# fab-jul/imgcomp-cvpr

Measured on AMD Instinct MI355X. Metric: Megapixels/s encode+pc-logits (and decode) per node, higher is better.
Workload: dtype f32

## Files before the change

### imgcomp_cvpr_amd/_lib.py

```python
import ctypes
import os
from ctypes import c_char_p, c_float, c_int, c_int64, c_longlong, c_size_t, c_uint32, c_void_p, POINTER

_HERE = os.path.dirname(os.path.abspath(__file__))
LIB_PATH = os.environ.get('IMGCOMP_HIP_LIB') or os.path.join(_HERE, 'libimgcomp_hip.so')


class HipLibraryError(RuntimeError):
    pass


CONV3_FORM_MASK = 0x0f
CONV3_AUTO, CONV3_DIRECT, CONV3_WINO, CONV3_WINO_WHOLEK, CONV3_WINO_WHOLEK_PW = 0, 1, 2, 3, 4
CONV3_WINO_KSPLIT, CONV3_WINO_T16, CONV3_WINO_SEG1, CONV3_WINO_SEG2, CONV3_WINO_SEG3 = 5, 6, 7, 8, 9
CONV3_WINO_PAIR = 10
CONV3_WINO4 = 11
CONV3_NO_WINO4 = 0x800000
CONV3_WINO4_WG8 = 0x8000000
CONV3_WINO4_WG4 = 0x10000000
CONV5_BOTH_PACKED = 0x1000000
CONV5_WINO4 = 0x2000000
CONV5_NO_WINO4 = 0x4000000
CONV3_LEAVE_IDLE_CUS = 0x10
CONV3_NO_XCD_RUNS = 0x20
CONV3_PACKED_TRANSFORM = 0x40
CONV3_STACK_KERNEL = 0x80


def CONV3_IN_FLIGHT(n):
    return (min(int(n), 15) & 0xf) << 19
PC_DECODE_PER_LAYER = 0x01
PC_DECODE_RECOMPUTE = 0x02
PC_DECODE_WAVEFRONT = 0x04


def conv3_leave_idle_layers(n):
    return (n & 0x7f) << 12


def conv3_direct_variant(v):
    return ((v + 1) & 0xf) << 8


def edge_tiles_per_wg(n):
    return n & 0xff


class PcTile(ctypes.Structure):
    _fields_ = [('y0', c_int), ('x0', c_int), ('th', c_int), ('tw', c_int), ('stream_off', c_longlong), ('stream_bytes', c_longlong),
                ('first_sym', c_int), ('volume', c_int)]


class PcVolume(ctypes.Structure):
    _fields_ = [('h', c_int), ('w', c_int), ('symbols_off', c_longlong), ('q_off', c_longlong)]


class PcSeg(ctypes.Structure):
    _fields_ = [('off', c_longlong), ('nbytes', c_longlong)]


def seg_table(segs):
    arr = (PcSeg * max(len(segs), 1))()
    for i, (off, n) in enumerate(segs):
        arr[i] = PcSeg(int(off), int(n))
    return arr


def tile_table(tiles):
    arr = (PcTile * len(tiles))()
    for i, t in enumerate(tiles):
        t = [int(v) for v in t]
        arr[i] = PcTile(*(t if len(t) == 8 else t + [0]))
    return arr


def volume_table(volumes):
    arr = (PcVolume * len(volumes))()
    for i, v in enumerate(volumes):
        arr[i] = PcVolume(*[int(x) for x in v])
    return arr


def packed_volume_table(shapes):
    offs, total = [], 0
    for C, h, w in shapes:
        offs.append(total)
        total += int(C) * int(h) * int(w)
    return volume_table([(h, w, o, o) for (C, h, w), o in zip(shapes, offs)]), offs, total


PROTOTYPES = {
    'ic_abi_version': (c_int, []),
    'ic_strerror': (c_char_p, [c_int]),
    'ic_crc32c': (c_uint32, [c_void_p, c_size_t, c_uint32]),
    'ic_conv2d_bn_act_f32': (c_int, [c_void_p] * 7 + [c_int] * 9 + [c_void_p, c_void_p, c_void_p]),
    'ic_deconv2d_bn_act_f32': (c_int, [c_void_p] * 5 + [c_int] * 8 + [c_void_p, c_void_p, c_int, c_void_p]),
    'ic_conv3x3_c128_packed_floats': (c_size_t, []),
    'ic_pack_conv3x3_c128_f32': (c_int, [c_void_p, c_void_p, c_void_p]),
    'ic_conv3x3_c128_bn_act_f32': (c_int, [c_void_p] * 7 + [c_int] * 5 + [c_void_p]),
    'ic_wino3x3_c128_packed_floats': (c_size_t, []),
    'ic_pack_wino3x3_c128_f32': (c_int, [c_void_p, c_void_p, c_int, c_void_p]),
    'ic_pack_wino3x3_c128_batch_f32': (c_int, [c_void_p, c_void_p, c_int, c_int, c_void_p]),
    'ic_wino3x3_c128_bn_act_f32': (c_int, [c_void_p] * 7 + [c_int] * 5 + [c_void_p]),
    'ic_wino3x3_c128_workgroups': (c_longlong, [c_int, c_int, c_int, c_int]),
    'ic_wino3x3_c128_plan': (c_int, [c_int, c_int, c_int, c_int, POINTER(c_longlong)]),
    'ic_conv3x3_c128_both_packed_floats': (c_size_t, []),
    'ic_pack_conv3x3_c128_both_f32': (c_int, [c_void_p, c_void_p, c_int, c_void_p]),
    'ic_conv3x3_c128_pick_algo': (c_int, [c_int, c_int, c_int, c_int]),
    'ic_conv3x3_c128_auto_f32': (c_int, [c_void_p] * 7 + [c_int] * 5 + [c_void_p]),
    'ic_conv2d_mfma_packed_floats': (c_size_t, [c_int] * 6),
    'ic_pack_conv2d_mfma_f32': (c_int, [c_void_p, c_void_p] + [c_int] * 6 + [c_void_p]),
    'ic_conv2d_mfma_bn_act_f32': (c_int, [c_void_p] * 5 + [c_int] * 10 + [c_void_p]),
    'ic_quantize_f32': (c_int, [c_void_p, c_void_p, c_int, c_float, c_void_p, c_void_p, c_void_p,
                                c_longlong, c_void_p]),
    'ic_heatmap_quantize_f32': (c_int, [c_void_p, c_void_p, c_int, c_float] + [c_void_p] * 6 +
                                [c_int] * 4 + [c_void_p]),
    'ic_pc_workspace_bytes': (c_size_t, [c_int] * 5),
    'ic_pc_packed_floats': (c_size_t, [c_int, c_int]),
    'ic_pc_mid_tile': (c_int, [c_int, c_int, c_int]),
    'ic_pc_pack_filters_f32': (c_int, [POINTER(c_void_p), c_int, c_int, c_void_p, c_void_p]),
    'ic_pc_logits_f32': (c_int, [c_void_p, POINTER(c_void_p), c_int, c_int, c_float, c_void_p] +
                         [c_int] * 4 + [c_void_p, c_size_t, c_void_p]),
    'ic_pc_logits_padded_f32': (c_int, [c_void_p, POINTER(c_void_p), c_int, c_int, c_void_p] +
                                [c_int] * 4 + [c_void_p, c_size_t, c_void_p]),
    'ic_pc_bitcost_f32': (c_int, [c_void_p, c_void_p, POINTER(c_void_p), c_int, c_int, c_float,
                                  c_void_p, c_void_p] + [c_int] * 4 + [c_void_p, c_size_t, c_void_p]),
    'ic_pc_logits_to_freqs_f32': (c_int, [c_void_p, c_longlong, c_int, c_float, c_void_p, c_void_p, c_void_p]),
    'ic_pc_encode_capacity_bytes': (c_size_t, [c_longlong]),
    'ic_pc_encode_f32': (c_int, [c_void_p, c_void_p, c_int, c_longlong, c_int, c_float, c_void_p, c_longlong, c_void_p, c_void_p,
                                 c_void_p]),
    'ic_pc_decode_workspace_bytes': (c_size_t, [c_int] * 4),
    'ic_pc_decode_f32': (c_int, [c_void_p, c_longlong, c_int, POINTER(c_void_p), c_void_p, c_int, c_int, c_float,
                                 c_void_p, c_void_p, c_int, c_int, c_int, c_void_p, c_size_t, c_int, c_void_p]),
    'ic_pc_decode_tiles_workspace_bytes': (c_size_t, [c_int] * 5),
    'ic_pc_decode_tiles_f32': (c_int, [c_void_p, c_longlong, c_void_p, c_int, POINTER(c_void_p), c_void_p, c_int, c_int, c_float,
                                       c_void_p, c_void_p, c_int, c_int, c_int, c_void_p, c_size_t, c_int, c_void_p]),
    'ic_pc_decode_tiles_batch_workspace_bytes': (c_size_t, [c_int] * 6),
    'ic_pc_decode_tiles_batch_f32': (c_int, [c_void_p, c_longlong, c_void_p, c_int, c_void_p, c_int, POINTER(c_void_p), c_void_p, c_int,
                                             c_int, c_float, c_void_p, c_void_p, c_void_p, c_int, c_void_p, c_size_t, c_int, c_void_p]),
    'ic_pc_decode_channels_f32': (c_int, [c_void_p, c_longlong, c_int, POINTER(c_void_p), c_void_p, c_int, c_int, c_float,
                                          c_void_p, c_void_p, c_int, c_int, c_int, c_void_p, c_size_t, c_int, c_void_p, c_int, c_int]),
    'ic_pc_decode_tiles_batch_channels_f32': (c_int, [c_void_p, c_longlong, c_void_p, c_int, c_void_p, c_int, POINTER(c_void_p), c_void_p,
                                                      c_int, c_int, c_float, c_void_p, c_void_p, c_void_p, c_int, c_void_p, c_size_t,
                                                      c_int, c_void_p, c_int, c_int]),
    'ic_pc_decode_tiles_batch_layers_workspace_bytes': (c_size_t, [c_int] * 7),
    'ic_pc_decode_tiles_batch_layers_f32': (c_int, [c_void_p, c_longlong, c_void_p, c_int, c_void_p, c_int, POINTER(c_void_p), c_void_p,
                                                    c_int, c_int, c_float, c_void_p, c_void_p, c_void_p, c_int, c_void_p, c_size_t,
                                                    c_int, c_void_p, c_int, c_int, c_void_p, c_int, c_void_p]),
    'ic_pc_encode_segments_f32': (c_int, [c_void_p, c_void_p, c_int, c_longlong, c_int, c_float, c_void_p, c_int, c_void_p, c_longlong,
                                          c_void_p, c_void_p, c_void_p]),
    'ic_pc_conceal_tiles_workspace_bytes': (c_size_t, [c_int, c_int, c_longlong]),
    'ic_pc_conceal_tiles': (c_int, [c_void_p, c_void_p, c_void_p, c_int, c_void_p, c_int, c_void_p, c_void_p] + [c_int] * 5 +
                            [c_void_p, c_size_t, c_void_p]),
    'ic_sum_f32': (c_int, [c_void_p, c_longlong, c_void_p, c_void_p, c_void_p]),
    'ic_mean_f32': (c_int, [c_void_p, c_longlong, c_float, c_void_p, c_void_p, c_void_p]),
    'ic_mean_rows_f32': (c_int, [c_void_p, c_int, c_longlong, c_float, c_void_p, c_void_p, c_void_p]),
    'ic_ae_workspace_bytes': (c_size_t, [c_int] * 4),
    'ic_ae_sync_pos_bytes': (c_size_t, [c_int] * 4),
    'ic_ae_res_stack_sync_pos_bytes': (c_size_t, [c_int] * 3),
    'ic_ae_encode_f32': (c_int, [c_void_p, POINTER(c_void_p)] + [c_int] * 5 + [c_void_p] * 6 +
                         [c_int] * 3 + [c_void_p, c_size_t, c_int, c_void_p]),
    'ic_ae_decode_f32': (c_int, [c_void_p, POINTER(c_void_p)] + [c_int] * 3 + [c_void_p] +
                         [c_int] * 3 + [c_void_p, c_size_t, c_int, c_void_p]),
    'ic_ae_res_stack_workspace_bytes': (c_size_t, [c_int] * 3),
    'ic_ae_res_stack_f32': (c_int, [c_void_p, POINTER(c_void_p), c_int, c_void_p] + [c_int] * 3 + [c_void_p, c_size_t, c_int, c_void_p]),
    'ic_peer_region_bytes': (c_size_t, []),
    'ic_peer_max_values': (c_int, []),
    'ic_peer_max_world': (c_int, []),
    'ic_peer_region_create': (c_int, [c_void_p, c_void_p]),
    'ic_peer_region_open': (c_int, [c_void_p, c_void_p]),
    'ic_peer_region_close': (c_int, [c_void_p]),
    'ic_peer_region_destroy': (c_int, [c_void_p]),
    'ic_peer_allreduce_f64': (c_int, [c_void_p, c_int, c_void_p, c_int, c_int, c_uint32, c_void_p, c_void_p]),
    'ic_build_has_tuning_forms': (c_int, []),
    'ic_conv3x3_c128_pick_form': (c_int, [c_int, c_int, c_int, c_int]),
    'ic_wino4_3x3_c128_packed_floats': (c_size_t, []),
    'ic_pack_wino4_3x3_c128_f32': (c_int, [c_void_p, c_void_p, c_int, c_void_p]),
    'ic_pack_wino4_3x3_c128_batch_f32': (c_int, [c_void_p, c_void_p, c_int, c_int, c_void_p]),
    'ic_wino4_3x3_c128_supported': (c_int, [c_int, c_int, c_int]),
# ... 116 lines not shown
```

### imgcomp_cvpr_amd/csrc/conv_edge.hip

```cpp
#include "internal.h"
#include <algorithm>

#define DE_TX 32
#define DE_TY 8

template <int CO>
__global__ __launch_bounds__(256) void deconv5_small_cout_kernel(const ConvArgs a) {
    extern __shared__ __attribute__((aligned(16))) float wl[];
    const int tid = threadIdx.x;
    const int n = blockIdx.z;
    for (int e = tid; e < a.Cin * 25 * 4; e += 256) {
        const int co = e & 3, tap = (e >> 2) % 25, ci = e / 100;
        wl[e] = co < a.Cout ? a.w[((size_t)tap * a.Cout + co) * a.Cin + ci] : 0.f;
    }
    __syncthreads();
    const int qx = blockIdx.x * DE_TX + (tid & (DE_TX - 1));
    const int qy = blockIdx.y * DE_TY + tid / DE_TX;
    const bool live = qx < a.W && qy < a.H;
    const int cx = min(qx, a.W - 1), cy = min(qy, a.H - 1);
    const int HW = a.H * a.W;
    const float* __restrict__ xin = a.x + (size_t)n * a.Cin * HW;
    int noff[9];
    bool nok[9];
#pragma unroll
// ... 112 lines not shown

#pragma unroll
    for (int c = 0; c < NCH; ++c) {
        e_f32x4 A[9][4];
#pragma unroll
        for (int t = 0; t < 9; ++t)
#pragma unroll
            for (int q = 0; q < 4; ++q)
                A[t][q] = *reinterpret_cast<const e_f32x4*>(wl + (size_t)t * 128 * CIN + 32 * c + 4 * q);
        if (c == 0) __syncthreads();
        float bv[2][4];
        auto views = [&](int s, int buf) __attribute__((always_inline)) {
            const float* Ls = L + (32 * c + s) * D3_CS;
            bv[buf][0] = Ls[0]; bv[buf][1] = Ls[-1]; bv[buf][2] = Ls[-D3_S]; bv[buf][3] = Ls[-D3_S - 1];
        };
        views(0, 0);
#pragma unroll
        for (int s = 0; s < 16; ++s) {
            if (s + 1 < 16) views(s + 1, (s + 1) & 1);
            const float b00 = bv[s & 1][0], b0m = bv[s & 1][1], bm0 = bv[s & 1][2], bmm = bv[s & 1][3];
#define D3_A(t) A[t][s >> 2][s & 3]
            p00a = __builtin_amdgcn_mfma_f32_32x32x2f32(D3_A(0), b00, p00a, 0, 0, 0);
            p01 = __builtin_amdgcn_mfma_f32_32x32x2f32(D3_A(1), b00, p01, 0, 0, 0);
            p10 = __builtin_amdgcn_mfma_f32_32x32x2f32(D3_A(3), b00, p10, 0, 0, 0);
            p11 = __builtin_amdgcn_mfma_f32_32x32x2f32(D3_A(4), b00, p11, 0, 0, 0);
            p00b = __builtin_amdgcn_mfma_f32_32x32x2f32(D3_A(2), b0m, p00b, 0, 0, 0);
            p10 = __builtin_amdgcn_mfma_f32_32x32x2f32(D3_A(5), b0m, p10, 0, 0, 0);
            p00a = __builtin_amdgcn_mfma_f32_32x32x2f32(D3_A(6), bm0, p00a, 0, 0, 0);
            p01 = __builtin_amdgcn_mfma_f32_32x32x2f32(D3_A(7), bm0, p01, 0, 0, 0);
            p00b = __builtin_amdgcn_mfma_f32_32x32x2f32(D3_A(8), bmm, p00b, 0, 0, 0);
#undef D3_A
#pragma unroll
            for (int i = 0; i < 9; ++i) {
                __builtin_amdgcn_sched_group_barrier(0x008, 1, 0);
                if (i < 4 && s + 1 < 16) __builtin_amdgcn_sched_group_barrier(0x100, 1, 0);
            }
        }
        __builtin_amdgcn_sched_barrier(0);
    }

    const int gy = gy0 + j / D3_TC, gx = gx0 + j % D3_TC;
    if (gy >= a.H || gx >= a.W) return;
    const size_t ohw = (size_t)a.OH * a.OW;
    float* __restrict__ yb = a.y + ((size_t)n * a.Cout + 32 * wave + 4 * kh) * ohw + (size_t)(2 * gy) * a.OW + 2 * gx;
    const float* __restrict__ scp = a.scale + 32 * wave + 4 * kh;
    const float* __restrict__ shp = a.shift + 32 * wave + 4 * kh;
#pragma unroll
    for (int r = 0; r < 16; ++r) {
        const int crow = (r & 3) + 8 * (r >> 2);
        const float sc = scp[crow], sh = shp[crow];
        float2 o0, o1;
        o0.x = fmaf(p00a[r] + p00b[r], sc, sh); o0.y = fmaf(p01[r], sc, sh);
        o1.x = fmaf(p10[r], sc, sh); o1.y = fmaf(p11[r], sc, sh);
        if (a.relu) {
            o0.x = fmaxf(o0.x, 0.f); o0.y = fmaxf(o0.y, 0.f); o1.x = fmaxf(o1.x, 0.f); o1.y = fmaxf(o1.y, 0.f);
        }
        float* dst = yb + (size_t)crow * ohw;
        *reinterpret_cast<float2*>(dst) = o0;
        *reinterpret_cast<float2*>(dst + a.OW) = o1;
    }
}

int icx_deconv3_mfma(const ConvArgs& a, hipStream_t st) {
    if (a.KH != 3 || a.KW != 3 || a.Cout != 128 || a.pt != 0 || a.pl != 0 || a.res1 || a.res2 || a.in_mean ||
        a.out_mean || a.builtin_norm || a.w_sci != 1 || a.w_sco != a.Cin)
        return IC_ERR_UNSUPPORTED;
    if ((long long)a.Cin * a.H * a.W >= (1ll << 31)) return IC_ERR_UNSUPPORTED;
    const int tiles_x = ic_cdiv(a.W, D3_TC), tiles_y = ic_cdiv(a.H, D3_TR);
    const dim3 g((unsigned)(tiles_x * tiles_y * a.N));
    if (a.Cin == 32) hipLaunchKernelGGL((deconv3_mfma_kernel<32>), g, dim3(256), 0, st, a, tiles_x, tiles_y);
    else if (a.Cin == 64) hipLaunchKernelGGL((deconv3_mfma_kernel<64>), g, dim3(256), 0, st, a, tiles_x, tiles_y);
    else return IC_ERR_UNSUPPORTED;
    IC_LAUNCH_CHECK();
    return IC_OK;
}

#define H1_TR 4
#define H1_TC 32
#define H1_ROWS ((H1_TR - 1) * 2 + 6)
#define H1_COLS ((H1_TC - 1) * 2 + 5)
#define H1_HALF ((H1_COLS + 1) / 2)
#define H1_S (2 * H1_HALF)
#define H1_CS (H1_ROWS * H1_S)

__global__ __launch_bounds__(256) void conv5s2_cin3_mfma_kernel(const ConvArgs a, int tiles_x, int tiles_y) {
    constexpr int NE = 3 * H1_ROWS * H1_COLS, NST = (NE + 255) / 256;
    __shared__ float lds[3 * H1_CS];
    __shared__ __attribute__((aligned(16))) float wl[25 * 3 * 64];
    const int tid = threadIdx.x, lane = tid & 63, wave = tid >> 6;
    int b = ic_xcd_run(blockIdx.x, gridDim.x);
    const int tx = b % tiles_x; b /= tiles_x;
    const int ty = b % tiles_y; const int n = b / tiles_y;
    const int ox0 = tx * H1_TC, oy0 = ty * H1_TR;
    const int HW = a.H * a.W;
    const float* __restrict__ xin = a.x + (size_t)n * 3 * HW;
    const int iy0 = 2 * oy0 - a.pt, ix0 = 2 * ox0 - a.pl;
    const bool norm_in = a.in_mean != nullptr || (a.builtin_norm & 1);

#pragma unroll
    for (int i = 0; i < NST; ++i) {
        const int e = tid + 256 * i;
        const int ci = e / (H1_ROWS * H1_COLS), rem = e - ci * (H1_ROWS * H1_COLS);
        const int rr = rem / H1_COLS, cc = rem - rr * H1_COLS;
        const int iy = iy0 + rr, ix = ix0 + cc;
        const bool live = e < NE;
        const bool ok = live && iy >= 0 && iy < a.H && ix >= 0 && ix < a.W;
        float v = xin[ok ? ci * HW + iy * a.W + ix : 0];
        if (norm_in) {
            const int cm = live ? ci : 0;
            const float m = a.in_mean ? a.in_mean[cm] : IC_IMG_MEAN[cm];
            const float s = a.in_mean ? a.in_std[cm] : IC_IMG_STD[cm];
            v = (v - m) / s;
        }
        if (live) lds[ci * H1_CS + rr * H1_S + (cc & 1) * H1_HALF + (cc >> 1)] = ok ? v : 0.f;
    }

    for (int e = tid; e < 25 * 3 * 64 / 4; e += 256)
        reinterpret_cast<float4*>(wl)[e] = reinterpret_cast<const float4*>(a.w)[e];
    __syncthreads();

    const int j = lane & 31, kh = lane >> 5;
    const float* __restrict__ L = lds + (2 * wave + kh) * H1_S + j;
    e_f32x16 acc0, acc1;
#pragma unroll
    for (int r = 0; r < 16; ++r) { acc0[r] = 0.f; acc1[r] = 0.f; }
    float fa[2][2], fb[2];
    auto operands = [&](int s, int buf) __attribute__((always_inline)) {
        const int ci = s / 15, p = (s / 5) % 3, kx = s % 5;
        const int ky = 2 * p + kh;
        const float* wp = wl + (((p < 2 ? ky : 4) * 5 + kx) * 3 + ci) * 64 + j;
        const float w0 = wp[0], w1 = wp[32];
        fa[buf][0] = (p < 2 || kh == 0) ? w0 : 0.f;
        fa[buf][1] = (p < 2 || kh == 0) ? w1 : 0.f;
        fb[buf] = L[ci * H1_CS + 2 * p * H1_S + (kx & 1) * H1_HALF + (kx >> 1)];
    };
    operands(0, 0);
#pragma unroll
    for (int s = 0; s < 45; ++s) {
        if (s + 1 < 45) operands(s + 1, (s + 1) & 1);
        acc0 = __builtin_amdgcn_mfma_f32_32x32x2f32(fa[s & 1][0], fb[s & 1], acc0, 0, 0, 0);
        acc1 = __builtin_amdgcn_mfma_f32_32x32x2f32(fa[s & 1][1], fb[s & 1], acc1, 0, 0, 0);
        __builtin_amdgcn_sched_group_barrier(0x008, 1, 0);
        __builtin_amdgcn_sched_group_barrier(0x100, 2, 0);
        __builtin_amdgcn_sched_group_barrier(0x008, 1, 0);
        __builtin_amdgcn_sched_group_barrier(0x100, 1, 0);
        __builtin_amdgcn_sched_group_barrier(0x002, 2, 0);
    }
    __builtin_amdgcn_sched_barrier(0);

    const int gy = oy0 + wave, gx = ox0 + j;
    if (gy >= a.OH || gx >= a.OW) return;
    const size_t ohw = (size_t)a.OH * a.OW;
    const size_t cs = a.out_phases ? ohw / 4 : ohw;
    const size_t o0 = a.out_phases ? (((size_t)n * 4 + 2 * (gy & 1) + (gx & 1)) * 64 + 4 * kh) * cs + (size_t)(gy >> 1) * (a.OW >> 1) + (gx >> 1)
                                   : ((size_t)n * 64 + 4 * kh) * ohw + (size_t)gy * a.OW + gx;
#pragma unroll
    for (int t = 0; t < 2; ++t)
#pragma unroll
        for (int r = 0; r < 16; ++r) {
            const int co = 32 * t + (r & 3) + 8 * (r >> 2);
            float v = fmaf(t ? acc1[r] : acc0[r], a.scale[co + 4 * kh], a.shift[co + 4 * kh]);
            if (a.relu) v = fmaxf(v, 0.f);
            const size_t o = o0 + (size_t)co * cs;
            if (a.res1) v += a.res1[o];
            if (a.res2) v += a.res2[o];
            a.y[o] = v;
        }
}

int icx_conv5s2_cin3_mfma(const ConvArgs& a, hipStream_t st) {
    if (a.KH != 5 || a.KW != 5 || a.stride != 2 || a.Cin != 3 || a.Cout != 64 || a.w_sco != 1 || a.w_sci != 64 ||
        a.out_mean || (a.builtin_norm & ~1))
        return IC_ERR_UNSUPPORTED;
    if ((long long)a.H * a.W * 3 >= (1ll << 31)) return IC_ERR_UNSUPPORTED;
    if (a.out_phases && ((a.OH | a.OW) & 1 || a.res1 || a.res2)) return IC_ERR_UNSUPPORTED;
    const int tiles_x = ic_cdiv(a.OW, H1_TC), tiles_y = ic_cdiv(a.OH, H1_TR);
    hipLaunchKernelGGL(conv5s2_cin3_mfma_kernel, dim3((unsigned)(tiles_x * tiles_y * a.N)), dim3(256), 0, st, a, tiles_x,
                       tiles_y);
    IC_LAUNCH_CHECK();
    return IC_OK;
}

typedef float e_f32x4v __attribute__((ext_vector_type(4)));
#define H13_TR 8
#define H13_TC 16
#define H13_S (H13_TC + 8)
#define H13_CS ((H13_TR + 2) * H13_S)
#define H13_KC 16
#define H13_UNITS (H13_KC * (H13_TR + 2) * (H13_S / 4))

__global__ __launch_bounds__(256) void deconv5_cout3_mfma_kernel(const ConvArgs a, int tiles_x, int tiles_y, int tpw,
                                                                 unsigned long long* prof) {
#ifdef H13_PROF
    unsigned long long tq[8], tp[4];
    tq[0] = __builtin_amdgcn_s_memtime();
#endif
    constexpr int NCH = 64 / H13_KC;
    constexpr unsigned OOB = 0x80000000u;
    __shared__ float af[16 * 9 * 64];
    __shared__ __attribute__((aligned(16))) float tl[2][H13_KC * H13_CS];
    const int tid = threadIdx.x, lane = tid & 63;
    const int wave = __builtin_amdgcn_readfirstlane(tid >> 6);
    const int strips = (tiles_x + tpw - 1) / tpw;
    int b = ic_xcd_run(blockIdx.x, gridDim.x);
    const int sx = b % strips; b /= strips;
    const int ty = b % tiles_y; const int n = b / tiles_y;
    const int tx0 = sx * tpw, nt = min(tpw, tiles_x - tx0);
    const int gy0 = ty * H13_TR;
    const int HW = a.H * a.W;
    const int j = lane & 15, kg = lane >> 4;
#ifdef H13_PROF
    __builtin_amdgcn_sched_barrier(0);
    tp[3] = __builtin_amdgcn_s_memtime() + (unsigned long long)(nt + HW == -12345);
    __builtin_amdgcn_sched_barrier(0);
#endif
    const __amdgpu_buffer_rsrc_t xr =
        __builtin_amdgcn_make_buffer_rsrc((void*)(a.x + (size_t)n * 64 * HW), 0, 64 * HW * 4, 0x00020000);
    const __amdgpu_buffer_rsrc_t wr = __builtin_amdgcn_make_buffer_rsrc((void*)a.w, 0, 25 * a.Cout * 64 * 4, 0x00020000);

    constexpr int NU = (H13_UNITS + 255) / 256;
    int ubase[NU], ulds[NU], ucol[NU];
#pragma unroll
    for (int i = 0; i < NU; ++i) {
        const int u = tid + 256 * i;
        const int sl = u / 60, rem = u - sl * 60;
        const int row = rem / 6, q = rem - row * 6;
        const int iy = gy0 - 1 + row;
        const bool ok = u < H13_UNITS && iy >= 0 && iy < a.H;
        ubase[i] = ok ? (16 * (sl & 3) + (sl >> 2)) * HW + iy * a.W : -1;
        ucol[i] = 4 * q - 4;
        ulds[i] = u < H13_UNITS ? sl * H13_CS + row * H13_S + 4 * q : -1;
    }
    unsigned voff[NU], vmask = 0;
    auto tile_off = [&](int gx0) {
        vmask = 0;
#pragma unroll
        for (int i = 0; i < NU; ++i) {
            const int ix = gx0 + ucol[i];
            voff[i] = ubase[i] >= 0 && ix >= 0 && ix < a.W ? (unsigned)(ubase[i] + ix) * 4u : OOB;
            const int left = a.W - ix;
            vmask |= (left >= 4 ? 15u : (1u << max(left, 0)) - 1u) << (4 * i);
        }
    };
    auto request = [&](e_f32x4* dst, int chunk) {
        const int cb = chunk * 4 * HW * 4;
#pragma unroll
        for (int i = 0; i < NU; ++i) dst[i] = __builtin_bit_cast(e_f32x4, __builtin_amdgcn_raw_buffer_load_b128(xr, voff[i], cb, 0));
    };
    auto deposit = [&](float* dstl, const e_f32x4* src, unsigned m) {
#pragma unroll
        for (int i = 0; i < NU; ++i) {
            e_f32x4 v = src[i];
#pragma unroll
            for (int e = 0; e < 4; ++e) v[e] = (m >> (4 * i + e)) & 1 ? v[e] : 0.f;
            if (i + 1 < NU || ulds[i] >= 0) *reinterpret_cast<e_f32x4*>(dstl + ulds[i]) = v;
        }
    };

    e_f32x4 fv[9];
    {
        const int i = lane & 15, co = i >> 2, py = (i >> 1) & 1, px = i & 1;
        const int tapf = a.Cout * 64;
        const unsigned lbase = co < a.Cout ? (unsigned)((((py + 1) * 5 + px + 1) * a.Cout + co) * 64 + 16 * kg + 4 * wave) * 4u : OOB;
// ... 158 lines not shown
```

### include/imgcomp_hip.h

```cpp
#ifndef IMGCOMP_HIP_H
#define IMGCOMP_HIP_H

#include <stddef.h>
#include <stdint.h>

#ifdef __cplusplus
extern "C" {
#endif

#define IC_ABI_VERSION 2

#define IC_OK 0
#define IC_ERR_ARG (-1)
#define IC_ERR_UNSUPPORTED (-2)
#define IC_ERR_WORKSPACE (-3)

typedef void* ic_stream_t;

#define IC_CONV3_FORM_MASK        0x0f
#define IC_CONV3_AUTO             0x00
#define IC_CONV3_DIRECT           0x01
#define IC_CONV3_WINO             0x02
#define IC_CONV3_WINO_WHOLEK      0x03
#define IC_CONV3_WINO_WHOLEK_PW   0x04
#define IC_CONV3_WINO_KSPLIT      0x05
#define IC_CONV3_WINO_T16         0x06
#define IC_CONV3_WINO_SEG1        0x07
#define IC_CONV3_WINO_SEG2        0x08
#define IC_CONV3_WINO_SEG3        0x09
#define IC_CONV3_WINO_PAIR        0x0a
#define IC_CONV3_WINO4            0x0b
#define IC_CONV3_NO_WINO4         0x800000
#define IC_CONV3_WINO4_WG8        0x8000000
#define IC_CONV3_WINO4_WG4        0x10000000
#define IC_CONV3_WINO4_BITS       (IC_CONV3_WINO4_WG8 | IC_CONV3_WINO4_WG4)
#define IC_CONV5_BOTH_PACKED      0x1000000
#define IC_CONV5_WINO4            0x2000000
#define IC_CONV5_NO_WINO4         0x4000000
int ic_build_has_tuning_forms(void);
#define IC_CONV3_LEAVE_IDLE_CUS   0x10
#define IC_CONV3_LEAVE_IDLE_LAYERS(n) (((n) & 0x7f) << 12)
#define IC_CONV3_NO_XCD_RUNS      0x20
#define IC_CONV3_STACK_KERNEL      0x80
#define IC_CONV3_PACKED_TRANSFORM 0x40
#define IC_CONV3_IN_FLIGHT(n)     (((n) & 0xf) << 19)
#define IC_CONV3_DIRECT_VARIANT(v) ((((v) + 1) & 0xf) << 8)
#define IC_EDGE_TILES_PER_WG(n)   ((n) & 0xff)
#define IC_PC_DECODE_PER_LAYER    0x01
#define IC_PC_DECODE_RECOMPUTE    0x02
#define IC_PC_DECODE_WAVEFRONT    0x04

int ic_abi_version(void);
const char* ic_strerror(int code);

uint32_t ic_crc32c(const void* host_data, size_t bytes, uint32_t crc);

int ic_conv2d_bn_act_f32(const float* x, const float* w, const float* scale, const float* shift,
                         const float* res1, const float* res2, float* y,
                         int N, int Cin, int H, int W, int Cout, int KH, int KW, int stride, int relu,
                         const float* in_mean, const float* in_std, ic_stream_t stream);

int ic_deconv2d_bn_act_f32(const float* x, const float* w, const float* scale, const float* shift,
                           float* y, int N, int Cin, int H, int W, int Cout, int KH, int KW, int relu,
                           const float* out_mean, const float* out_std, int flags, ic_stream_t stream);

size_t ic_conv3x3_c128_packed_floats(void);
int ic_pack_conv3x3_c128_f32(const float* w_tf, float* w_packed, ic_stream_t stream);
int ic_conv3x3_c128_bn_act_f32(const float* x, const float* w_packed, const float* scale,
                               const float* shift, const float* res1, const float* res2, float* y,
                               int N, int H, int W, int relu, int flags, ic_stream_t stream);

size_t ic_wino3x3_c128_packed_floats(void);
int ic_pack_wino3x3_c128_f32(const float* w_tf, float* w_packed, int backward, ic_stream_t stream);
int ic_pack_wino3x3_c128_batch_f32(const float* const* w_tf_table_dev, float* w_packed, int layers, int backward,
                                   ic_stream_t stream);
int ic_wino3x3_c128_bn_act_f32(const float* x, const float* w_packed, const float* scale,
                               const float* shift, const float* res1, const float* res2, float* y,
                               int N, int H, int W, int relu, int flags, ic_stream_t stream);
long long ic_wino3x3_c128_workgroups(int N, int H, int W, int flags);
int ic_wino3x3_c128_plan(int N, int H, int W, int flags, long long plan_out[5]);

size_t ic_conv3x3_c128_both_packed_floats(void);
int ic_pack_conv3x3_c128_both_f32(const float* w_tf, float* w_packed, int backward, ic_stream_t stream);
int ic_conv3x3_c128_pick_algo(int N, int H, int W, int flags);
int ic_conv3x3_c128_auto_f32(const float* x, const float* w_both, const float* scale, const float* shift,
                             const float* res1, const float* res2, float* y, int N, int H, int W, int relu,
                             int flags, ic_stream_t stream);

size_t ic_conv2d_mfma_packed_floats(int KH, int KW, int Cin, int Cout, int stride, int transposed);
int ic_pack_conv2d_mfma_f32(const float* w_tf, float* w_packed, int KH, int KW, int Cin, int Cout,
                            int stride, int transposed, ic_stream_t stream);
int ic_conv2d_mfma_bn_act_f32(const float* x, const float* w_packed, const float* scale, const float* shift,
                              float* y, int N, int Cin, int H, int W, int Cout, int KH, int KW, int stride,
                              int transposed, int relu, ic_stream_t stream);

int ic_quantize_f32(const float* z, const float* centers, int L, float sigma,
                    float* qsoft, float* qhard, int64_t* symbols, long long count, ic_stream_t stream);
int ic_heatmap_quantize_f32(const float* bottleneck, const float* centers, int L, float sigma,
                            float* heatmap, float* z, float* qsoft, float* qhard, float* qbar,
                            int64_t* symbols, int N, int C, int h, int w, ic_stream_t stream);

size_t ic_pc_workspace_bytes(int N, int C, int h, int w, int k);
size_t ic_pc_packed_floats(int k, int L);
int ic_pc_pack_filters_f32(const float* const* wtab_host, int k, int L, float* packed, ic_stream_t stream);
int ic_pc_mid_tile(int k, int OH, int OW);
int ic_pc_logits_f32(const float* q, const float* const* wtab_host, int k, int L, float pad_value,
                     float* logits, int N, int C, int h, int w,
                     void* workspace, size_t workspace_bytes, ic_stream_t stream);
int ic_pc_logits_padded_f32(const float* vol, const float* const* wtab_host, int k, int L,
                            float* logits, int N, int D, int H, int W,
                            void* workspace, size_t workspace_bytes, ic_stream_t stream);
int ic_pc_bitcost_f32(const float* q, const int64_t* symbols, const float* const* wtab_host, int k, int L,
                      float pad_value, float* logits, float* bits, int N, int C, int h, int w,
                      void* workspace, size_t workspace_bytes, ic_stream_t stream);
int ic_pc_logits_to_freqs_f32(const float* logits, long long count, int L, float resolution,
                              int64_t* freqs, float* pr, ic_stream_t stream);

size_t ic_pc_decode_workspace_bytes(int C, int h, int w, int k);
int ic_pc_decode_f32(const uint8_t* bitstream, long long nbytes, int first_sym, const float* const* wtab_host,
                     const float* centers, int k, int L, float resolution, int64_t* symbols, int* status,
                     int C, int h, int w, void* workspace, size_t workspace_bytes, int flags, ic_stream_t stream);
typedef struct { int y0, x0, th, tw; long long stream_off, stream_bytes; int first_sym, volume; } ic_pc_tile_t;
size_t ic_pc_decode_tiles_workspace_bytes(int C, int th_max, int tw_max, int ntiles, int k);
int ic_pc_decode_tiles_f32(const uint8_t* bitstreams, long long total_bytes, const ic_pc_tile_t* tiles_host, int ntiles,
                           const float* const* wtab_host, const float* centers, int k, int L, float resolution,
                           int64_t* symbols, int* status, int C, int h, int w, void* workspace, size_t workspace_bytes,
                           int flags, ic_stream_t stream);
typedef struct { int h, w; long long symbols_off, q_off; } ic_pc_volume_t;
size_t ic_pc_decode_tiles_batch_workspace_bytes(int C, int th_max, int tw_max, int ntiles, int nvolumes, int k);
int ic_pc_decode_tiles_batch_f32(const uint8_t* bitstreams, long long total_bytes, const ic_pc_tile_t* tiles_host, int ntiles,
                                 const ic_pc_volume_t* volumes_host, int nvolumes, const float* const* wtab_host,
                                 const float* centers, int k, int L, float resolution, int64_t* symbols, float* q, int* status,
                                 int C, void* workspace, size_t workspace_bytes, int flags, ic_stream_t stream);
int ic_pc_decode_channels_f32(const uint8_t* bitstream, long long nbytes, int first_sym, const float* const* wtab_host,
                              const float* centers, int k, int L, float resolution, int64_t* symbols, int* status,
                              int C, int h, int w, void* workspace, size_t workspace_bytes, int flags, ic_stream_t stream,
                              int channels, int fill_sym);
int ic_pc_decode_tiles_batch_channels_f32(const uint8_t* bitstreams, long long total_bytes, const ic_pc_tile_t* tiles_host, int ntiles,
                                          const ic_pc_volume_t* volumes_host, int nvolumes, const float* const* wtab_host,
                                          const float* centers, int k, int L, float resolution, int64_t* symbols, float* q,
                                          int* status, int C, void* workspace, size_t workspace_bytes, int flags,
                                          ic_stream_t stream, int channels, int fill_sym);
typedef struct { long long off, nbytes; } ic_pc_seg_t;
size_t ic_pc_decode_tiles_batch_layers_workspace_bytes(int C, int th_max, int tw_max, int ntiles, int nvolumes, int k, int nlayers);
int ic_pc_decode_tiles_batch_layers_f32(const uint8_t* bitstreams, long long total_bytes, const ic_pc_tile_t* tiles_host, int ntiles,
                                        const ic_pc_volume_t* volumes_host, int nvolumes, const float* const* wtab_host,
                                        const float* centers, int k, int L, float resolution, int64_t* symbols, float* q,
// ... 151 lines not shown
```

Measured before the change: 243.4.

## Process multiple x-tiles per workgroup in first conv with prefetched buffer loads

The first 5x5 stride-2 conv (Cin=3) kernel now walks a strip of several horizontal tiles per workgroup, prefetching the next tile's input with 128-bit buffer loads while computing the current one. Weights are staged into shared memory once per strip instead of once per tile. Output goes through a shared-memory transpose so that stores and residual reads are 4-wide. A heuristic picks tiles per workgroup while keeping at least 768 workgroups, and a new C entry point exposes the kernel with a tune field. The cost is more shared memory (an extra 16KB output buffer), which may lower occupancy, and a tighter size limit on supported inputs.

After: 242.5. No clear change (-0.4%).

```diff
diff --git a/imgcomp_cvpr_amd/_lib.py b/imgcomp_cvpr_amd/_lib.py
--- a/imgcomp_cvpr_amd/_lib.py
+++ b/imgcomp_cvpr_amd/_lib.py
@@ -95,6 +95,7 @@
     'ic_crc32c': (c_uint32, [c_void_p, c_size_t, c_uint32]),
     'ic_conv2d_bn_act_f32': (c_int, [c_void_p] * 7 + [c_int] * 9 + [c_void_p, c_void_p, c_void_p]),
     'ic_deconv2d_bn_act_f32': (c_int, [c_void_p] * 5 + [c_int] * 8 + [c_void_p, c_void_p, c_int, c_void_p]),
+    'ic_conv5s2_cin3_bn_act_f32': (c_int, [c_void_p] * 5 + [c_int] * 4 + [c_void_p, c_void_p, c_int, c_int, c_void_p]),
     'ic_conv3x3_c128_packed_floats': (c_size_t, []),
     'ic_pack_conv3x3_c128_f32': (c_int, [c_void_p, c_void_p, c_void_p]),
     'ic_conv3x3_c128_bn_act_f32': (c_int, [c_void_p] * 7 + [c_int] * 5 + [c_void_p]),
diff --git a/imgcomp_cvpr_amd/csrc/conv_edge.hip b/imgcomp_cvpr_amd/csrc/conv_edge.hip
--- a/imgcomp_cvpr_amd/csrc/conv_edge.hip
+++ b/imgcomp_cvpr_amd/csrc/conv_edge.hip
@@ -218,103 +218,191 @@
 #define H1_HALF ((H1_COLS + 1) / 2)
 #define H1_S (2 * H1_HALF)
 #define H1_CS (H1_ROWS * H1_S)
-
-__global__ __launch_bounds__(256) void conv5s2_cin3_mfma_kernel(const ConvArgs a, int tiles_x, int tiles_y) {
-    constexpr int NE = 3 * H1_ROWS * H1_COLS, NST = (NE + 255) / 256;
+#define H1_NQ 18
+#define H1_UNITS (3 * H1_ROWS * H1_NQ)
+
+typedef float e_f32x4u __attribute__((ext_vector_type(4), aligned(4)));
+
+__global__ __launch_bounds__(256) void conv5s2_cin3_mfma_kernel(const ConvArgs a, int tiles_x, int tiles_y, int tpw) {
+    constexpr int NU = (H1_UNITS + 255) / 256;
+    constexpr unsigned OOB = 0x80000000u;
     __shared__ float lds[3 * H1_CS];
     __shared__ __attribute__((aligned(16))) float wl[25 * 3 * 64];
+    __shared__ __attribute__((aligned(16))) float ol[4 * 32 * 32];
     const int tid = threadIdx.x, lane = tid & 63, wave = tid >> 6;
+    const int strips = (tiles_x + tpw - 1) / tpw;
     int b = ic_xcd_run(blockIdx.x, gridDim.x);
-    const int tx = b % tiles_x; b /= tiles_x;
+    const int sx = b % strips; b /= strips;
     const int ty = b % tiles_y; const int n = b / tiles_y;
-    const int ox0 = tx * H1_TC, oy0 = ty * H1_TR;
+    const int tx0 = sx * tpw, nt = min(tpw, tiles_x - tx0);
+    const int oy0 = ty * H1_TR;
     const int HW = a.H * a.W;
-    const float* __restrict__ xin = a.x + (size_t)n * 3 * HW;
-    const int iy0 = 2 * oy0 - a.pt, ix0 = 2 * ox0 - a.pl;
+    const int iy0 = 2 * oy0 - a.pt;
     const bool norm_in = a.in_mean != nullptr || (a.builtin_norm & 1);
-
-#pragma unroll
-    for (int i = 0; i < NST; ++i) {
-        const int e = tid + 256 * i;
-        const int ci = e / (H1_ROWS * H1_COLS), rem = e - ci * (H1_ROWS * H1_COLS);
-        const int rr = rem / H1_COLS, cc = rem - rr * H1_COLS;
-        const int iy = iy0 + rr, ix = ix0 + cc;
-        const bool live = e < NE;
-        const bool ok = live && iy >= 0 && iy < a.H && ix >= 0 && ix < a.W;
-        float v = xin[ok ? ci * HW + iy * a.W + ix : 0];
-        if (norm_in) {
-            const int cm = live ? ci : 0;
-            const float m = a.in_mean ? a.in_mean[cm] : IC_IMG_MEAN[cm];
-            const float s = a.in_mean ? a.in_std[cm] : IC_IMG_STD[cm];
-            v = (v - m) / s;
-        }
-        if (live) lds[ci * H1_CS + rr * H1_S + (cc & 1) * H1_HALF + (cc >> 1)] = ok ? v : 0.f;
-    }
+    const __amdgpu_buffer_rsrc_t xr =
+        __builtin_amdgcn_make_buffer_rsrc((void*)(a.x + (size_t)n * 3 * HW), 0, 3 * HW * 4, 0x00020000);
+
+    int ubase[NU], ulds[NU], ucc[NU];
+    float um[NU], us[NU];
+#pragma unroll
+    for (int i = 0; i < NU; ++i) {
+        const int u = tid + 256 * i;
+        const bool live = u < H1_UNITS;
+        const int ci = u / (H1_ROWS * H1_NQ), rem = u - ci * (H1_ROWS * H1_NQ);
+        const int rr = rem / H1_NQ, q = rem - rr * H1_NQ;
+        const int iy = iy0 + rr;
+        ubase[i] = live && iy >= 0 && iy < a.H ? ci * HW + iy * a.W : -1;
+        ucc[i] = live ? 4 * q - 4 + a.pl : -1024;
+        ulds[i] = live ? ci * H1_CS + rr * H1_S : 0;
+        const int cm = live ? ci : 0;
+        um[i] = a.in_mean ? a.in_mean[cm] : IC_IMG_MEAN[cm];
+        us[i] = a.in_mean ? a.in_std[cm] : IC_IMG_STD[cm];
+    }
+    e_f32x4 st[NU];
+    auto request = [&](int tx) {
+#pragma unroll
+        for (int i = 0; i < NU; ++i) {
+            const int ix = 64 * tx - a.pl + ucc[i];
+            const unsigned voff = ubase[i] >= 0 && ix >= 0 && ix < a.W ? (unsigned)(ubase[i] + ix) * 4u : OOB;
+            st[i] = __builtin_bit_cast(e_f32x4, __builtin_amdgcn_raw_buffer_load_b128(xr, voff, 0, 0));
+        }
+    };
+    auto deposit = [&](int tx) {
+#pragma unroll
+        for (int i = 0; i < NU; ++i)
+#pragma unroll
+            for (int e = 0; e < 4; ++e) {
+                const int cc = ucc[i] + e, ix = 64 * tx - a.pl + cc;
+                const bool ok = ubase[i] >= 0 && ix >= 0 && ix < a.W;
+                float v = st[i][e];
+                if (norm_in) v = (v - um[i]) / us[i];
+                if (cc >= 0 && cc < H1_COLS) lds[ulds[i] + (cc & 1) * H1_HALF + (cc >> 1)] = ok ? v : 0.f;
+            }
+    };
+    request(tx0);
 
     for (int e = tid; e < 25 * 3 * 64 / 4; e += 256)
         reinterpret_cast<float4*>(wl)[e] = reinterpret_cast<const float4*>(a.w)[e];
-    __syncthreads();
 
     const int j = lane & 31, kh = lane >> 5;
     const float* __restrict__ L = lds + (2 * wave + kh) * H1_S + j;
-    e_f32x16 acc0, acc1;
-#pragma unroll
-    for (int r = 0; r < 16; ++r) { acc0[r] = 0.f; acc1[r] = 0.f; }
-    float fa[2][2], fb[2];
-    auto operands = [&](int s, int buf) __attribute__((always_inline)) {
-        const int ci = s / 15, p = (s / 5) % 3, kx = s % 5;
-        const int ky = 2 * p + kh;
-        const float* wp = wl + (((p < 2 ? ky : 4) * 5 + kx) * 3 + ci) * 64 + j;
-        const float w0 = wp[0], w1 = wp[32];
-        fa[buf][0] = (p < 2 || kh == 0) ? w0 : 0.f;
-        fa[buf][1] = (p < 2 || kh == 0) ? w1 : 0.f;
-        fb[buf] = L[ci * H1_CS + 2 * p * H1_S + (kx & 1) * H1_HALF + (kx >> 1)];
-    };
-    operands(0, 0);
-#pragma unroll
-    for (int s = 0; s < 45; ++s) {
-        if (s + 1 < 45) operands(s + 1, (s + 1) & 1);
-        acc0 = __builtin_amdgcn_mfma_f32_32x32x2f32(fa[s & 1][0], fb[s & 1], acc0, 0, 0, 0);
-        acc1 = __builtin_amdgcn_mfma_f32_32x32x2f32(fa[s & 1][1], fb[s & 1], acc1, 0, 0, 0);
-        __builtin_amdgcn_sched_group_barrier(0x008, 1, 0);
-        __builtin_amdgcn_sched_group_barrier(0x100, 2, 0);
-        __builtin_amdgcn_sched_group_barrier(0x008, 1, 0);
-        __builtin_amdgcn_sched_group_barrier(0x100, 1, 0);
-        __builtin_amdgcn_sched_group_barrier(0x002, 2, 0);
-    }
-    __builtin_amdgcn_sched_barrier(0);
-
-    const int gy = oy0 + wave, gx = ox0 + j;
-    if (gy >= a.OH || gx >= a.OW) return;
+    float* __restrict__ ow = ol + wave * (32 * 32);
+    const int jo = a.out_phases ? (j & 1) * 16 + (j >> 1) : j;
+    const int q8 = lane & 7, cr = lane >> 3;
+    const int gy = oy0 + wave;
     const size_t ohw = (size_t)a.OH * a.OW;
     const size_t cs = a.out_phases ? ohw / 4 : ohw;
-    const size_t o0 = a.out_phases ? (((size_t)n * 4 + 2 * (gy & 1) + (gx & 1)) * 64 + 4 * kh) * cs + (size_t)(gy >> 1) * (a.OW >> 1) + (gx >> 1)
-                                   : ((size_t)n * 64 + 4 * kh) * ohw + (size_t)gy * a.OW + gx;
-#pragma unroll
-    for (int t = 0; t < 2; ++t)
-#pragma unroll
-        for (int r = 0; r < 16; ++r) {
-            const int co = 32 * t + (r & 3) + 8 * (r >> 2);
-            float v = fmaf(t ? acc1[r] : acc0[r], a.scale[co + 4 * kh], a.shift[co + 4 * kh]);
-            if (a.relu) v = fmaxf(v, 0.f);
-            const size_t o = o0 + (size_t)co * cs;
-            if (a.res1) v += a.res1[o];
-            if (a.res2) v += a.res2[o];
-            a.y[o] = v;
-        }
-}
-
+    const int roww = a.out_phases ? a.OW >> 1 : a.OW;
+    const size_t obase = a.out_phases ? ((size_t)n * 4 + 2 * (gy & 1) + (q8 >> 2)) * 64 * cs + (size_t)(gy >> 1) * roww
+                                      : (size_t)n * 64 * cs + (size_t)gy * roww;
+
+    for (int tile = 0; tile < nt; ++tile) {
+        const int tx = tx0 + tile;
+        deposit(tx);
+        __syncthreads();
+        if (tile + 1 < nt) request(tx + 1);
+        __builtin_amdgcn_sched_barrier(0);
+
+        e_f32x16 acc0, acc1;
+#pragma unroll
+        for (int r = 0; r < 16; ++r) { acc0[r] = 0.f; acc1[r] = 0.f; }
+        float fa[2][2], fb[2];
+        auto operands = [&](int s, int buf) __attribute__((always_inline)) {
+            const int ci = s / 15, p = (s / 5) % 3, kx = s % 5;
+            const int ky = 2 * p + kh;
+            const float* wp = wl + (((p < 2 ? ky : 4) * 5 + kx) * 3 + ci) * 64 + j;
+            const float w0 = wp[0], w1 = wp[32];
+            fa[buf][0] = (p < 2 || kh == 0) ? w0 : 0.f;
+            fa[buf][1] = (p < 2 || kh == 0) ? w1 : 0.f;
+            fb[buf] = L[ci * H1_CS + 2 * p * H1_S + (kx & 1) * H1_HALF + (kx >> 1)];
+        };
+        operands(0, 0);
+#pragma unroll
+        for (int s = 0; s < 45; ++s) {
+            if (s + 1 < 45) operands(s + 1, (s + 1) & 1);
+            acc0 = __builtin_amdgcn_mfma_f32_32x32x2f32(fa[s & 1][0], fb[s & 1], acc0, 0, 0, 0);
+            acc1 = __builtin_amdgcn_mfma_f32_32x32x2f32(fa[s & 1][1], fb[s & 1], acc1, 0, 0, 0);
+            __builtin_amdgcn_sched_group_barrier(0x008, 1, 0);
+            __builtin_amdgcn_sched_group_barrier(0x100, 2, 0);
+            __builtin_amdgcn_sched_group_barrier(0x008, 1, 0);
+            __builtin_amdgcn_sched_group_barrier(0x100, 1, 0);
+            __builtin_amdgcn_sched_group_barrier(0x002, 2, 0);
+        }
+        __builtin_amdgcn_sched_barrier(0);
+
+        const int col = (a.out_phases ? 16 * tx + 4 * (q8 & 3) : 32 * tx + 4 * q8), left = roww - col;
+#pragma unroll
+        for (int t = 0; t < 2; ++t) {
+#pragma unroll
+            for (int r = 0; r < 16; ++r) ow[((r & 3) + 8 * (r >> 2) + 4 * kh) * 32 + jo] = t ? acc1[r] : acc0[r];
+            __syncthreads();
+#pragma unroll
+            for (int i = 0; i < 4; ++i) {
+                const int co = 32 * t + 8 * i + cr;
+                e_f32x4 v = *reinterpret_cast<const e_f32x4*>(ow + (8 * i + cr) * 32 + 4 * q8);
+                const float sc = a.scale[co], sh = a.shift[co];
+#pragma unroll
+                for (int e = 0; e < 4; ++e) {
+                    v[e] = fmaf(v[e], sc, sh);
+                    if (a.relu) v[e] = fmaxf(v[e], 0.f);
+                }
+                if (gy >= a.OH || left <= 0) continue;
+                const size_t o = obase + (size_t)co * cs + col;
+                if (left >= 4) {
+                    if (a.res1) v += *reinterpret_cast<const e_f32x4u*>(a.res1 + o);
+                    if (a.res2) v += *reinterpret_cast<const e_f32x4u*>(a.res2 + o);
+                    *reinterpret_cast<e_f32x4u*>(a.y + o) = v;
+                } else {
+#pragma unroll
+                    for (int e = 0; e < 3; ++e) {
+                        if (e >= left) break;
+                        float s = v[e];
+                        if (a.res1) s += a.res1[o + e];
+                        if (a.res2) s += a.res2[o + e];
+                        a.y[o + e] = s;
+                    }
+                }
+            }
+            __syncthreads();
+        }
+    }
+}
+
+static int h1_auto_tpw(int tiles_x, int tiles_y, int N) {
+    int tpw = 1;
+    for (int cand = 2; cand <= std::min(tiles_x, 8); ++cand)
+        if ((long long)ic_cdiv(tiles_x, cand) * tiles_y * N >= 768) tpw = cand;
+    return tpw;
+}
 int icx_conv5s2_cin3_mfma(const ConvArgs& a, hipStream_t st) {
     if (a.KH != 5 || a.KW != 5 || a.stride != 2 || a.Cin != 3 || a.Cout != 64 || a.w_sco != 1 || a.w_sci != 64 ||
-        a.out_mean || (a.builtin_norm & ~1))
+        a.out_mean || (a.builtin_norm & ~1) || a.pl < 0 || a.pl > 4)
         return IC_ERR_UNSUPPORTED;
-    if ((long long)a.H * a.W * 3 >= (1ll << 31)) return IC_ERR_UNSUPPORTED;
+    if ((long long)a.H * a.W * 3 >= (1ll << 29)) return IC_ERR_UNSUPPORTED;
     if (a.out_phases && ((a.OH | a.OW) & 1 || a.res1 || a.res2)) return IC_ERR_UNSUPPORTED;
     const int tiles_x = ic_cdiv(a.OW, H1_TC), tiles_y = ic_cdiv(a.OH, H1_TR);
-    hipLaunchKernelGGL(conv5s2_cin3_mfma_kernel, dim3((unsigned)(tiles_x * tiles_y * a.N)), dim3(256), 0, st, a, tiles_x,
-                       tiles_y);
+    int tpw = a.tune;
+    if (tpw <= 0) tpw = h1_auto_tpw(tiles_x, tiles_y, a.N);
+    tpw = std::min(tpw, tiles_x);
+    const int strips = ic_cdiv(tiles_x, tpw);
+    tpw = ic_cdiv(tiles_x, strips);
+    hipLaunchKernelGGL(conv5s2_cin3_mfma_kernel, dim3((unsigned)(strips * tiles_y * a.N)), dim3(256), 0, st, a, tiles_x,
+                       tiles_y, tpw);
     IC_LAUNCH_CHECK();
     return IC_OK;
+}
+
+extern "C" int ic_conv5s2_cin3_bn_act_f32(const float* x, const float* w, const float* scale, const float* shift, float* y,
+                                          int N, int H, int W, int relu, const float* in_mean, const float* in_std,
+                                          int out_phases, int flags, ic_stream_t stream) {
+    IC_CHECK_ARG(x && w && scale && shift && y && N > 0 && H > 0 && W > 0);
+    IC_CHECK_ARG((in_mean == nullptr) == (in_std == nullptr));
+    ConvArgs a{};
+    a.x = x; a.w = w; a.scale = scale; a.shift = shift; a.y = y; a.in_mean = in_mean; a.in_std = in_std;
+    a.N = N; a.Cin = 3; a.H = H; a.W = W; a.Cout = 64; a.KH = 5; a.KW = 5; a.stride = 2; a.relu = relu;
+    a.out_phases = out_phases ? 1 : 0;
+    a.tune = flags & 0xff;
+    return icx_conv2d(a, false, (hipStream_t)stream);
 }
 
 typedef float e_f32x4v __attribute__((ext_vector_type(4)));
diff --git a/include/imgcomp_hip.h b/include/imgcomp_hip.h
--- a/include/imgcomp_hip.h
+++ b/include/imgcomp_hip.h
@@ -63,6 +63,10 @@
 int ic_deconv2d_bn_act_f32(const float* x, const float* w, const float* scale, const float* shift,
                            float* y, int N, int Cin, int H, int W, int Cout, int KH, int KW, int relu,
                            const float* out_mean, const float* out_std, int flags, ic_stream_t stream);
+
+int ic_conv5s2_cin3_bn_act_f32(const float* x, const float* w, const float* scale, const float* shift, float* y,
+                               int N, int H, int W, int relu, const float* in_mean, const float* in_std,
+                               int out_phases, int flags, ic_stream_t stream);
 
 size_t ic_conv3x3_c128_packed_floats(void);
 int ic_pack_conv3x3_c128_f32(const float* w_tf, float* w_packed, ic_stream_t stream);
```
